# daultanigaurav/AI-BASED-FRAME-INTERPOLATION

Hardware: AMD Instinct MI355X
Metric: interpolated frames/sec at 1080p (higher is better)
Workload: dtype bf16

## Files before the change

ai_based_frame_interpolation_amd/_native.py:

```python
from __future__ import annotations

import ctypes
import os
import subprocess

import torch

_PKG = os.path.dirname(os.path.abspath(__file__))
LIB_PATH = os.environ.get("FIUNET_LIB") or os.path.join(_PKG, "libfiunet_hip.so")
CSRC = os.path.join(_PKG, "csrc")

ABI_VERSION = 8
ABI_MIN_COMPAT = 4
FP32, BF16, BF16X2, FP16 = 0, 1, 2, 3
OPT_UNFUSED, OPT_KEEP_ALL, OPT_GATHER_UPSAMPLE = 1, 2, 16
OPT_RNE_WEIGHTS, OPT_NO_DITHER = 32, 64
WEIGHT_PREPS = ("host", "device")
YUV_MPEG2, YUV_BT709, YUV_FULL_RANGE, YUV_BT2020 = 1, 2, 4, 8

SYMBOLS = (
    "fiunet_abi_version", "fiunet_last_error_string", "fiunet_create", "fiunet_destroy",
    "fiunet_set_options", "fiunet_load_weights", "fiunet_load_weights_device", "fiunet_prepare_precision", "fiunet_workspace_bytes", "fiunet_forward",
    "fiunet_min_unsplit_batch",
    "fiunet_forward_strip",
    "fiunet_workspace_bytes_u8", "fiunet_forward_u8", "fiunet_forward_u8_strided", "fiunet_preprocess_u8",
    "fiunet_postprocess_u8", "fiunet_debug_read_activation", "fiunet_profile_enable",
    "fiunet_profile_read", "fiunet_metrics_workspace_bytes", "fiunet_psnr_u8", "fiunet_ssim_u8",
    "fiunet_ssim_gauss_workspace_bytes", "fiunet_ssim_gauss_f32",
    "fiunet_plane_metrics_workspace_bytes", "fiunet_plane_psnr", "fiunet_plane_ssim",
    "fiunet_interleaved_psnr", "fiunet_stepped_ssim",
    "fiunet_yuv420_to_rgb_u8", "fiunet_rgb_to_yuv420_u8", "fiunet_workspace_bytes_yuv420", "fiunet_forward_yuv420",
# ... 794 lines not shown
```

ai_based_frame_interpolation_amd/csrc/conv3x3_mfma.hip.h:

```cpp
#pragma once
#include "conv_common.hip.h"

namespace fiunet {

template <typename T, int BN, int TH, int TW, int MODE, int EPI>
__global__ __launch_bounds__(256, conv_occupancy(BN, TH, TW, ConvTile<BN, TH, TW, MODE>::LDS_BYTES)) void conv3x3_mfma_kernel(const ConvArgs a)
{
    using Tile = ConvTile<BN, TH, TW, MODE>;
    constexpr int PL = Elem<T>::PL;
    constexpr int TWP = Tile::TWP, THP = Tile::THP;
    constexpr int WAVES_C = BN / 64, WAVES_P = 4 / WAVES_C;
    constexpr int FR = TW / 16;
    constexpr int NF = conv_wave_frags(BN, TH, TW);
    constexpr int ROWS_W = NF / FR;
    static_assert(NF == 8 || NF == 4, "wave tile must be 64 couts x 128 or 64 pixels");
    static_assert(TH == ROWS_W * WAVES_P && ROWS_W * FR == NF, "tile does not split over the waves");
    static_assert(EPI != EPI_POOL || ROWS_W % 2 == 0, "pooled epilogue: a wave owns whole row pairs");
    static_assert(Tile::LDS_BYTES * conv_occupancy(BN, TH, TW, Tile::LDS_BYTES) <= 160 * 1024, "LDS per CU");
    constexpr int HNC = EPI == EPI_HEAD ? 1 : (EPI == EPI_HEAD3 ? 3 : 0);
    static_assert(HNC == 0 || BN == 64, "fused head needs all 64 couts in one wave");
    static_assert(MODE == SRC_DIRECT || MODE == SRC_CONCAT_UP || MODE == SRC_STEM || MODE == SRC_DIRECT_X2 ||
                  MODE == SRC_STEM_X2, "pooling is fused into the producer");
    constexpr bool X2 = src_is_x2(MODE);
    constexpr bool STEM = src_is_stem(MODE);
    constexpr bool DIRECT = MODE == SRC_DIRECT || MODE == SRC_DIRECT_X2;
    static_assert(!X2 || std::is_same_v<T, __bf16>, "two-piece operands are bf16");
    static_assert(!STEM || (sizeof(T) == 2 && BN == 64), "fused stem: 2-byte output (bf16 / fp16), 64 couts");

    extern __shared__ __attribute__((aligned(16))) char smem[];
    char* const lds_in = smem;
    char* const lds_w = smem + Tile::IN_BYTES;
// ... 30 lines not shown
#define STAMP(slot) do {} while (0)
#define STAMP_UP(slot) do {} while (0)
#define PSTAMP(slot) do {} while (0)
#endif
    f32x4 acc[4][NF];
    conv_acc_init<T, BN, TH, TW, EPI>(a, acc, ct, wc, lc);
#ifdef FIUNET_STAMP_PROLOG
    asm volatile("" :: "v"(acc[3][NF - 1][3]), "v"(acc[0][0][0]));
#endif
    PSTAMP(9);

    const int a_off = (wc * 64 + l15) * 64 + ((lc ^ swz(l15)) << 4);
    int b_off[3];
#pragma unroll
    for (int kx = 0; kx < 3; ++kx)
        b_off[kx] = (wp * ROWS_W * TWP + kx + l15) * 64 + ((lc ^ swz(kx + l15)) << 4);

    const int nplanes_real = (a.C0 + a.C1) / PL;
    const int nplanes_all = X2 ? 3 * nplanes_real : nplanes_real;
    const int p0 = a.C0 / PL;
    const int pbeg = split * nplanes_all / ksplit, pend = (split + 1) * nplanes_all / ksplit;
    const int nsteps = (pend - pbeg) * 3;
    const char* wbase = (const char*)a.wgt + (size_t)ct * BN * 64;

    constexpr int NW = Tile::W_BYTES / 1024 / 4;
    static_assert(BN % 16 == 0, "a weight piece must not straddle two taps");
    const unsigned w_lane_off = (unsigned)((lane >> 2) * 64 + (((lane & 3) ^ swz(lane >> 2)) << 4));
    auto issue_w = [&](int step) __attribute__((always_inline)) {
        const int lp = step / 3, kx = step - lp * 3;
        int pl = pbeg + lp;
        if constexpr (X2) {
// ... 12 lines not shown
#ifndef FIUNET_DIAG_FREE_PROLOGUE
    issue_w(0);
#endif
#ifdef FIUNET_DIAG_NO_WSTREAM
    if (nsteps > 1) issue_w(1);
#endif
    PSTAMP(10);

    constexpr int NPIECE = THP * TWP / 16;
    static_assert(THP * TWP % 16 == 0, "in-tile must be a whole number of 1-KiB pieces");
    const int aH = a.H, aW = a.W;
    const char* const dma_src = (const char*)a.src0 + (size_t)b * a.H * a.W * a.C0 * sizeof(T) * (X2 ? 2 : 1);
    const char* const dma_src1 = DIRECT && a.C1 > 0
                                     ? (const char*)a.src1 + (size_t)b * a.H * a.W * a.C1 * sizeof(T) * (X2 ? 2 : 1) : nullptr;
    constexpr bool HOIST = (MODE == SRC_DIRECT && BN == 128 && EPI == EPI_PLAIN) ||
                           (NF == 4 && DIRECT);
    constexpr bool ROLL = sizeof(T) == 2 && FR == 2 && (!epi_is_splitk(EPI) || NF == 4);
    constexpr int NPW = (NPIECE + 3) / 4;
    unsigned in_off[HOIST ? NPW : 1];
    const unsigned plane_bytes = (unsigned)(aH * aW) * 64u;
    unsigned pm_lin0 = 0, pm_valid = 0, pm_wrap = 0;
    static_assert(NPW <= 32, "one mask bit per piece of a wave");
    constexpr int PM_DY = 64 / TWP, PM_DX = 64 % TWP;
    const unsigned pm_dlin = (unsigned)(PM_DY * aW + PM_DX) * 64u, pm_dwrap = (unsigned)(aW - TWP) * 64u;
    if constexpr (!STEM) {
        const int row0 = wave * 16 + (lane >> 2);
        int py = row0 / TWP, px = row0 - py * TWP;
        int y = y0 - 1 + py, x = x0 - 1 + px;
        pm_lin0 = (unsigned)(y * aW + x) * 64u + (((lane & 3) ^ swz(row0)) << 4);
        unsigned lin = pm_lin0;
#pragma unroll
        for (int jj = 0; jj < NPW; ++jj) {
// ... 380 lines not shown
#endif
            const char* wcur = lds_w + (step & 1) * Tile::W_STRIDE + a_off;
            constexpr bool EARLY_OK = ROLL && DIRECT;
            bool early = false;
            if constexpr (EARLY_OK)
                early = kx == 2 && gather_next && (DIRECT || plane + 1 < p0);
            if constexpr (ROLL) {
                uint4 xb[ROWS_W + 2][FR];
                auto load_row = [&](int i) __attribute__((always_inline)) {
#pragma unroll
                    for (int f = 0; f < FR; ++f)
                        xb[i][f] = *reinterpret_cast<const uint4*>(lds_in + b_off[kx] + (i * TWP + f * 16) * 64);
                };
#pragma unroll
                for (int i = 0; i < ROWS_W; ++i) load_row(i);
#pragma unroll
                for (int ky = 0; ky < 3; ++ky) {
                    uint4 wa[4];
#pragma unroll
                    for (int m = 0; m < 4; ++m)
                        wa[m] = *reinterpret_cast<const uint4*>(wcur + (ky * BN + m * 16) * 64);
                    if (ky < 2) load_row(ROWS_W + ky);
                    if (ky == 1 && early) {
                        __syncthreads();
                        gather_plane(plane + 1, step & 1, false);
                    }
#pragma unroll
                    for (int m = 0; m < 4; ++m)
#pragma unroll
                        for (int n = 0; n < NF; ++n) mma_chunk<T>(acc[m][n], wa[m], xb[n / FR + ky][n % FR]);
                }
            } else {
#pragma unroll
                for (int ky = 0; ky < 3; ++ky) {
                    asm volatile("" ::: "memory");
                    uint4 wa[4], xb[NF];
#pragma unroll
                    for (int m = 0; m < 4; ++m)
                        wa[m] = *reinterpret_cast<const uint4*>(wcur + (ky * BN + m * 16) * 64);
#pragma unroll
                    for (int n = 0; n < NF; ++n)
                        xb[n] = *reinterpret_cast<const uint4*>(
                            lds_in + b_off[kx] + (((n / FR) + ky) * TWP + (n % FR) * 16) * 64);
#pragma unroll
                    for (int m = 0; m < 4; ++m)
// ... 23 lines not shown

#ifdef FIUNET_CLOCK
    {
        asm volatile("" :: "v"(acc[3][NF - 1][3]));
        __builtin_amdgcn_sched_barrier(0);
        const unsigned long long ck_t1 = __builtin_amdgcn_s_memtime(), ck_r1 = __builtin_amdgcn_s_memrealtime();
        const unsigned st_idx = blockIdx.x * 4u + (unsigned)wave;
        if (a.stamp && lane == 0 && st_idx < a.stamp_cap) {
            unsigned long long* rec = a.stamp + (size_t)st_idx * 16;
            rec[0] = ck_t1 - ck_t0;
            rec[1] = ck_r1 - ck_r0;
            rec[8] = 1ull;
        }
    }
#endif
    conv_epilogue<T, BN, TH, TW, EPI, X2>(a, acc, b, y0, x0, ct, split, wc, wp, l15, lc);
#ifdef FIUNET_STAMP
    STAMP(5);
    st_sum[0] = st_prev - st_t0;
    const unsigned st_idx = blockIdx.x * 4u + (unsigned)wave;
    if (a.stamp && lane == 0 && st_idx < a.stamp_cap) {
        unsigned long long* rec = a.stamp + (size_t)st_idx * 16;
#pragma unroll
        for (int k = 0; k < 16; ++k) rec[k] = k == 8 ? 1ull : st_sum[k];
    }
#endif
}

template <typename T, int BN, int TH, int TW, int EPI, bool X2>
__global__ __launch_bounds__(64) void splitk_finalize_tile_kernel(const ConvArgs a)
{
// ... 56 lines not shown
```

ai_based_frame_interpolation_amd/csrc/conv_common.hip.h:

```cpp
#pragma once
#include <hip/hip_runtime.h>
#include <stdint.h>
#include <type_traits>

namespace fiunet {

typedef __attribute__((ext_vector_type(4))) float f32x4;
typedef __attribute__((ext_vector_type(8))) __bf16 bf16x8;
typedef __attribute__((ext_vector_type(8))) _Float16 f16x8;

enum SrcMode { SRC_DIRECT = 0, SRC_POOL = 1 , SRC_CONCAT_UP = 2,
               SRC_STEM = 3 ,
               SRC_DIRECT_X2 = 4,
               SRC_STEM_X2 = 5 };
constexpr bool src_is_stem(int mode) { return mode == SRC_STEM || mode == SRC_STEM_X2; }
constexpr bool src_is_x2(int mode) { return mode == SRC_DIRECT_X2 || mode == SRC_STEM_X2; }

__device__ __forceinline__ size_t blk_off(int plane, int y, int x, int H, int W)
{
    return (((size_t)plane * H + y) * W + x) * 64;
}

struct ConvArgs {
    const void* src0;
// ... 374 lines not shown
    static constexpr int TAB_OFF = PATCH_OFF + ((PATCH_BYTES + 15) / 16) * 16;
    static constexpr int TAB_BYTES = MODE == SRC_CONCAT_UP ? ((THP + TW + 2) * 16 + 255) / 256 * 256 : 0;
    static constexpr int STEMW_OFF = TAB_OFF + TAB_BYTES;
    static constexpr int STEMW_BYTES = src_is_stem(MODE) ? 4096 : 0;
    static constexpr int LDS_BYTES = STEMW_OFF + STEMW_BYTES;
    static_assert(LDS_BYTES <= 80 * 1024, "two workgroups must fit in the CU's 160 KiB of LDS");
    static_assert(!src_is_stem(MODE) || LDS_BYTES <= 63 * 1280, "fused-stem kernel: stay below 64 LDS granules");
};

constexpr int conv_wave_frags(int BN, int TH, int TW) { return TH * TW / 16 / (4 / (BN / 64)); }
constexpr int conv_occupancy(int BN, int TH, int TW, int lds_bytes = 0)
{
    return conv_wave_frags(BN, TH, TW) == 4 && lds_bytes * 3 <= 160 * 1024 ? 3 : 2;
}


__device__ __forceinline__ int conv_block_remap()
{
    const int nblk = gridDim.x, bid = blockIdx.x;
    const int q = nblk >> 3, r = nblk & 7, xcd = bid & 7;
    return (xcd < r ? xcd * (q + 1) : r * (q + 1) + (xcd - r) * q) + (bid >> 3);
}

struct ConvTileId { int ct, b, ty, tx; };
__device__ __forceinline__ ConvTileId conv_tile_decode(const ConvArgs& a, int t)
{
    ConvTileId d;
    d.ct = t % a.nct; t /= a.nct;
    d.tx = t % a.tilesX; t /= a.tilesX;
    d.ty = t % a.tilesY;
// ... 18 lines not shown
            const float4 sh = *reinterpret_cast<const float4*>(a.shift + ct * BN + wc * 64 + conv_cout_ofs<T>(m, lc));
            v = f32x4{sh.x, sh.y, sh.z, sh.w};
        }
#pragma unroll
        for (int n = 0; n < NF; ++n) acc[m][n] = v;
    }
}

__device__ __forceinline__ unsigned relu_pk_bf16(unsigned p) { return pk_max_i16(p, 0u); }
__device__ __forceinline__ void relu_fma(float& sum, float x, float lo, float w)
{
    float t;
    asm("v_max_f32 %1, %3, %2\n\tv_fmac_f32 %0, %1, %4" : "+v"(sum), "=&v"(t) : "v"(x), "v"(lo), "v"(w));
}

template <typename T, int BN, int TH, int TW, int EPI, bool X2 = false>
__device__ __forceinline__ void conv_epilogue(const ConvArgs& a, f32x4 (&acc)[4][conv_wave_frags(BN, TH, TW)],
                                              int b, int y0, int x0, int ct, int split, int wc, int wp,
                                              int l15, int lc)
{
    constexpr int PL = Elem<T>::PL;
    constexpr int FR = TW / 16;
    constexpr int NF = conv_wave_frags(BN, TH, TW);
    constexpr int ROWS_W = NF / FR;
    constexpr int HNC = EPI == EPI_HEAD ? 1 : (EPI == EPI_HEAD3 ? 3 : 0);
    const int aH = a.H, aW = a.W;
    constexpr bool PERM = sizeof(T) == 2;
    const int wbase_c = ct * BN + wc * 64;
    if constexpr (epi_is_splitk(EPI)) {
        const int tile = (((b * a.tilesY) + y0 / TH) * a.tilesX + x0 / TW) * a.nct + ct;
        const int ntile = a.B * a.tilesY * a.tilesX * a.nct;
        const int wave = wp * (BN / 64) + wc;
        float4* o = reinterpret_cast<float4*>(a.kslab) + ((((size_t)split * ntile + tile) * 4 + wave) * (4 * NF)) * 64 + (lc * 16 + l15);
#pragma unroll
        for (int m = 0; m < 4; ++m)
#pragma unroll
            for (int n = 0; n < NF; ++n)
                o[(m * NF + n) * 64] = make_float4(acc[m][n][0], acc[m][n][1], acc[m][n][2], acc[m][n][3]);
        return;
    }
    float hw[HNC > 0 ? HNC : 1][4][4];
// ... 29 lines not shown
#pragma unroll
                for (int m = 0; m < 4; ++m)
#pragma unroll
                    for (int j = 0; j < 4; ++j) relu_fma(sum, acc[m][n][j], floor_v, hw[c][m][j]);
                hs[n] = sum;
            }
            if constexpr (NF == 4) {
                float full[NF];
#pragma unroll
                for (int n = 0; n < NF; ++n) {
                    const float p = hs[n] + __shfl_xor(hs[n], 16);
                    full[n] = p + __shfl_xor(p, 32);
                }
                const float mine = lc == 0 ? full[0] : (lc == 1 ? full[1] : (lc == 2 ? full[2] : full[3]));
                const int n = lc;
                const int y = y0 + wp * ROWS_W + n / FR;
                const int x = x0 + (n % FR) * 16 + l15;
                if (y < aH && x < aW) {
                    const size_t o = (size_t)b * a.head_img_stride + ((size_t)c * aH + y) * aW + x;
                    if (a.head_out_u8) a.head_out_u8[o] = postprocess_u8_value(mine + hb[c]);
                    else a.head_out[o] = mine + hb[c];
                }
            } else {
                float t[4], u[2];
#pragma unroll
                for (int i = 0; i < 4; ++i) {
                    const auto r = __builtin_amdgcn_permlane16_swap(__float_as_uint(hs[i]), __float_as_uint(hs[(i + 4) % NF]), false, false);
                    t[i] = __uint_as_float(r[0]) + __uint_as_float(r[1]);
                }
#pragma unroll
                for (int j = 0; j < 2; ++j) {
                    const auto r = __builtin_amdgcn_permlane32_swap(__float_as_uint(t[j]), __float_as_uint(t[j + 2]), false, false);
                    u[j] = __uint_as_float(r[0]) + __uint_as_float(r[1]);
                }
#pragma unroll
                for (int j = 0; j < 2; ++j) {
                    const int n = nb + j;
                    const int y = y0 + wp * ROWS_W + n / FR;
                    const int x = x0 + (n % FR) * 16 + l15;
                    if (y < aH && x < aW) {
                        const size_t o = (size_t)b * a.head_img_stride + ((size_t)c * aH + y) * aW + x;
                        if (a.head_out_u8) a.head_out_u8[o] = postprocess_u8_value(u[j] + hb[c]);
                        else a.head_out[o] = u[j] + hb[c];
                    }
                }
            }
        }
    }
    if constexpr (X2) {
        static_assert(std::is_same_v<T, __bf16>, "the two-piece epilogue belongs to the bf16 kernels");
        if (HNC > 0 && !a.dst) return;
        const size_t ps = (size_t)aH * aW * 64;
        const int npo = a.Cout / 32;
        const size_t blk = (size_t)npo * ps;
// ... 2 lines not shown
        const size_t pps = (size_t)pH2 * pW2 * 64, pblk = (size_t)npo * pps;
        char* const pimg = EPI == EPI_POOL ? (char*)a.pool_dst + (size_t)b * 2 * pblk + (size_t)(wbase_c / 32) * pps + lc * 16
                                           : nullptr;
        auto put = [&](char* o, size_t block_bytes, const float (&v)[8]) __attribute__((always_inline)) {
            unsigned h[4], l[4];
#pragma unroll
            for (int i = 0; i < 4; ++i) {
                h[i] = pack_bf16x2_pk(v[2 * i], v[2 * i + 1]);
                l[i] = pack_bf16x2_pk(v[2 * i] - __uint_as_float(h[i] << 16), v[2 * i + 1] - __uint_as_float(h[i] & 0xffff0000u));
            }
            *reinterpret_cast<uint4*>(o) = make_uint4(h[0], h[1], h[2], h[3]);
            *reinterpret_cast<uint4*>(o + block_bytes) = make_uint4(l[0], l[1], l[2], l[3]);
        };
#pragma unroll
        for (int n = 0; n < NF; ++n) {
            const int y = y0 + wp * ROWS_W + n / FR;
            const int x = x0 + (n % FR) * 16 + l15;
            if (y < aH && x < aW) {
#pragma unroll
                for (int g = 0; g < 2; ++g) {
                    float v[8];
#pragma unroll
                    for (int j = 0; j < 4; ++j) {
                        v[j] = a.relu ? fmaxf(acc[2 * g][n][j], 0.f) : acc[2 * g][n][j];
                        v[4 + j] = a.relu ? fmaxf(acc[2 * g + 1][n][j], 0.f) : acc[2 * g + 1][n][j];
                    }
                    put(img + (size_t)(y * aW + x) * 64 + g * ps, blk, v);
                }
            }
        }
        if constexpr (EPI == EPI_POOL) {
#pragma unroll
            for (int n = 0; n < NF; ++n) {
                if (((n / FR) & 1) != 0) continue;
                const int y = y0 + wp * ROWS_W + n / FR;
                const int x = x0 + (n % FR) * 16 + l15;
                const int py = y >> 1, px = x >> 1;
                const bool okp = (py < pH2) && (px < pW2) && ((l15 & 1) == 0);
#pragma unroll
                for (int g = 0; g < 2; ++g) {
                    float v[8];
#pragma unroll
                    for (int h = 0; h < 2; ++h)
#pragma unroll
                        for (int j = 0; j < 4; ++j) {
                            const float cm = fmaxf(acc[2 * g + h][n][j], acc[2 * g + h][n + FR][j]);
                            float r = fmaxf(cm, __uint_as_float(dpp_swap_pairs(__float_as_uint(cm))));
                            if (a.relu) r = fmaxf(r, 0.f);
                            v[4 * h + j] = r;
                        }
                    if (okp) put(pimg + (size_t)(min(py, pH2 - 1) * pW2 + min(px, pW2 - 1)) * 64 + g * pps, pblk, v);
                }
            }
        }
        return;
    }
    if constexpr (EPI == EPI_POOL && PERM) {
#pragma unroll
        for (int n = 0; n < NF; ++n) {
            if (((n / FR) & 1) != 0) continue;
            uint4 pk[2][2];
#pragma unroll
            for (int r = 0; r < 2; ++r) {
                const int nn = n + r * FR;
                const int y = y0 + wp * ROWS_W + nn / FR;
                const int x = x0 + (nn % FR) * 16 + l15;
                const bool ok = (y < aH) && (x < aW);
                char* o = out_img + (size_t)(y * aW + x) * 64;
#pragma unroll
                for (int g = 0; g < 2; ++g) {
                    uint4 v = make_uint4(pack2_pk<T>(acc[2 * g][nn][0], acc[2 * g][nn][1]),
                                         pack2_pk<T>(acc[2 * g][nn][2], acc[2 * g][nn][3]),
                                         pack2_pk<T>(acc[2 * g + 1][nn][0], acc[2 * g + 1][nn][1]),
                                         pack2_pk<T>(acc[2 * g + 1][nn][2], acc[2 * g + 1][nn][3]));
                    if (a.relu) v = make_uint4(relu_pk_bf16(v.x), relu_pk_bf16(v.y), relu_pk_bf16(v.z), relu_pk_bf16(v.w));
                    pk[r][g] = v;
                    if (ok && out_img) *reinterpret_cast<uint4*>(o + g * plane_stride) = v;
                }
            }
            const int y = y0 + wp * ROWS_W + n / FR;
            const int x = x0 + (n % FR) * 16 + l15;
            const int py = y >> 1, px = x >> 1;
            const bool okp = (py < pH) && (px < pW) && ((l15 & 1) == 0);
            char* o = pool_img + (size_t)(min(py, pH - 1) * pW + min(px, pW - 1)) * 64;
#pragma unroll
            for (int g = 0; g < 2; ++g) {
                const uint4 t = pk[0][g], u = pk[1][g];
                const unsigned c0 = pk_max_i16(t.x, u.x), c1 = pk_max_i16(t.y, u.y);
                const unsigned c2 = pk_max_i16(t.z, u.z), c3 = pk_max_i16(t.w, u.w);
                const uint4 m = make_uint4(pk_max_i16(c0, dpp_swap_pairs(c0)), pk_max_i16(c1, dpp_swap_pairs(c1)),
                                           pk_max_i16(c2, dpp_swap_pairs(c2)), pk_max_i16(c3, dpp_swap_pairs(c3)));
                if (okp) *reinterpret_cast<uint4*>(o + g * pplane_stride) = m;
            }
        }
        return;
    }
#pragma unroll
    for (int n = 0; n < NF; ++n) {
        const int y = y0 + wp * ROWS_W + n / FR;
        const int x = x0 + (n % FR) * 16 + l15;
        const bool ok = (y < aH) && (x < aW);
        if (ok && out_img) {
            char* o = out_img + (size_t)(y * aW + x) * 64;
            if constexpr (PERM) {
#pragma unroll
                for (int g = 0; g < 2; ++g) {
                    uint4 pk = make_uint4(pack2<T>(acc[2 * g][n][0], acc[2 * g][n][1]),
                                          pack2<T>(acc[2 * g][n][2], acc[2 * g][n][3]),
                                          pack2<T>(acc[2 * g + 1][n][0], acc[2 * g + 1][n][1]),
                                          pack2<T>(acc[2 * g + 1][n][2], acc[2 * g + 1][n][3]));
                    if (a.relu) pk = make_uint4(relu_pk_bf16(pk.x), relu_pk_bf16(pk.y), relu_pk_bf16(pk.z), relu_pk_bf16(pk.w));
                    *reinterpret_cast<uint4*>(o + g * plane_stride) = pk;
                }
            } else {
#pragma unroll
                for (int m = 0; m < 4; ++m) {
                    float4 v = make_float4(acc[m][n][0], acc[m][n][1], acc[m][n][2], acc[m][n][3]);
                    if (a.relu) v = make_float4(fmaxf(v.x, 0.f), fmaxf(v.y, 0.f), fmaxf(v.z, 0.f), fmaxf(v.w, 0.f));
                    *reinterpret_cast<float4*>(o + m * plane_stride) = v;
                }
            }
        }
    }
    if (EPI == EPI_POOL) {
#pragma unroll
        for (int n = 0; n < NF; ++n) {
            if (((n / FR) & 1) != 0) continue;
            const int y = y0 + wp * ROWS_W + n / FR;
            const int x = x0 + (n % FR) * 16 + l15;
            const int py = y >> 1, px = x >> 1;
            const bool okp = (py < pH) && (px < pW) && ((l15 & 1) == 0);
            char* o = pool_img + (size_t)(min(py, pH - 1) * pW + min(px, pW - 1)) * 64;
            if constexpr (!PERM) {
#pragma unroll
                for (int m = 0; m < 4; ++m) {
                    float r[4];
#pragma unroll
                    for (int j = 0; j < 4; ++j) {
                        const float cm = fmaxf(acc[m][n][j], acc[m][n + FR][j]);
                        r[j] = fmaxf(cm, __uint_as_float(dpp_swap_pairs(__float_as_uint(cm))));
                        if (a.relu) r[j] = fmaxf(r[j], 0.f);
                    }
                    if (okp) *reinterpret_cast<float4*>(o + m * pplane_stride) = make_float4(r[0], r[1], r[2], r[3]);
                }
// ... 24 lines not shown
```

ai_based_frame_interpolation_amd/csrc/conv_launch.hip.h:

```cpp
#pragma once
#include "fiunet_internal.h"
#include "conv3x3_kwave.hip.h"

#include <atomic>
#include <cstdio>

namespace fiunet {
namespace {

template <auto Kernel>
int launch_lds(const char* name, long long nblk, int lds, const ConvArgs& a, hipStream_t s)
{
    if (name_out()) *name_out() = name;
    if (nblk <= 0 || nblk > 0x7fffffffLL) return fail(FIUNET_ERR_INVALID_ARG, "conv grid too large");
    static std::atomic<bool> lds_attr_set[64];
    int dev = 0;
    HIP_TRY(hipGetDevice(&dev));
    if (dev >= 0 && dev < 64 && !lds_attr_set[dev].load(std::memory_order_acquire)) {
        HIP_TRY(hipFuncSetAttribute(reinterpret_cast<const void*>(Kernel), hipFuncAttributeMaxDynamicSharedMemorySize, lds));
        lds_attr_set[dev].store(true, std::memory_order_release);
    }
    hipLaunchKernelGGL(Kernel, dim3((unsigned)nblk), dim3(256), lds, s, a);
    HIP_TRY(hipGetLastError());
    return FIUNET_OK;
}

template <typename T, int BN, int TH, int TW, int MODE, int EPI>
int launch_conv_cfg(ConvArgs a, hipStream_t s)
{
    char name[128] = "";
    if (name_out())
        std::snprintf(name, sizeof name, "conv3x3_mfma_kernel<%s,%d,%d,%d,%d,%d>", elem_name<T>(), BN, TH, TW,
                      MODE, EPI);
    a.tilesX = (a.W + TW - 1) / TW;
    a.tilesY = (a.H + TH - 1) / TH;
    a.nct = a.Cout / BN;
    const long long nblk = (long long)a.B * a.tilesX * a.tilesY * a.nct * (epi_is_splitk(EPI) ? a.ksplit : 1);
    return launch_lds<&conv3x3_mfma_kernel<T, BN, TH, TW, MODE, EPI>>(name, nblk, ConvTile<BN, TH, TW, MODE>::LDS_BYTES, a, s);
}

template <typename T, int EPI, bool X2> int launch_kwave(ConvArgs a, hipStream_t s)
{
    using Tile = KWaveTile;
    char name[96] = "";
    if (name_out())
        std::snprintf(name, sizeof name, "conv3x3_kwave_kernel<%s%s,64,2,32,%d>+kwave4", elem_name<T>(), X2 ? "x2" : "", EPI);
    a.tilesX = (a.W + Tile::TW - 1) / Tile::TW;
    a.tilesY = (a.H + Tile::TH - 1) / Tile::TH;
    a.nct = a.Cout / Tile::BN;
    return launch_lds<&conv3x3_kwave_kernel<EPI, X2, T>>(name, (long long)a.B * a.tilesX * a.tilesY * a.nct, Tile::LDS_BYTES, a, s);
}

template <typename T, int BN, int TH, int TW, int MODE, int EPI>
// ... 14 lines not shown
            if (name_out()) *name_out() += "+splitk" + std::to_string(ksplit);
            return FIUNET_OK;
        }
    }
    return launch_conv_cfg<T, BN, TH, TW, MODE, EPI>(a, s);
}

template <typename T, int MODE, int EPI> int launch_conv_shape(const ConvArgs& a, const ConvCfg& cfg, hipStream_t s)
{
    if (a.Cout != 64 && a.Cout % 128 != 0) return fail(FIUNET_ERR_INVALID_ARG, "Cout must be 64 or k*128");
    if ((EPI == EPI_HEAD || EPI == EPI_HEAD3) && a.Cout != 64) return fail(FIUNET_ERR_INVALID_ARG, "fused head needs Cout == 64");
    if constexpr ((MODE == SRC_DIRECT || MODE == SRC_DIRECT_X2) && (EPI == EPI_PLAIN || EPI == EPI_POOL)) {
        if (cfg.kwave) return launch_kwave<T, EPI, MODE == SRC_DIRECT_X2>(a, s);
    }
    if (cfg.small) return launch_conv_maybe_split<T, 64, 8, 32, MODE, EPI>(a, s, cfg.ksplit);
    if (a.Cout == 64) {
        const bool wide = prefer_wide(a.H, a.W, 16, 32, 32, 16);
        return wide ? launch_conv_maybe_split<T, 64, 16, 32, MODE, EPI>(a, s, cfg.ksplit)
                    : launch_conv_maybe_split<T, 64, 32, 16, MODE, EPI>(a, s, cfg.ksplit);
    }
    if constexpr (EPI != EPI_HEAD && EPI != EPI_HEAD3) {
        const bool wide = prefer_wide(a.H, a.W, 8, 32, 16, 16);
        return wide ? launch_conv_maybe_split<T, 128, 8, 32, MODE, EPI>(a, s, cfg.ksplit)
                    : launch_conv_maybe_split<T, 128, 16, 16, MODE, EPI>(a, s, cfg.ksplit);
    }
    return fail(FIUNET_ERR_INVALID_ARG, "fused head needs Cout == 64");
}

}

template <typename T> int launch_conv(const ConvArgs& a, int mode, int epi, const ConvCfg& cfg, hipStream_t s)
{
    constexpr int PL = Elem<T>::PL;
    if (a.C0 % PL || a.C1 % PL) return fail(FIUNET_ERR_INVALID_ARG, "channels not a plane multiple");
    if (mode == SRC_CONCAT_UP && epi == EPI_PLAIN) return launch_conv_shape<T, SRC_CONCAT_UP, EPI_PLAIN>(a, cfg, s);
    if (mode == SRC_DIRECT && epi == EPI_PLAIN) return launch_conv_shape<T, SRC_DIRECT, EPI_PLAIN>(a, cfg, s);
    if (mode == SRC_DIRECT && epi == EPI_HEAD) return launch_conv_shape<T, SRC_DIRECT, EPI_HEAD>(a, cfg, s);
// ... 15 lines not shown
```

ai_based_frame_interpolation_amd/csrc/fiunet.hip:

```cpp
#include "fiunet_internal.h"
#include "pointwise.hip.h"
#include "weights.hip.h"

#include <cmath>
#include <cstdio>
#include <cstring>
#include <map>

using namespace fiunet;

namespace {

thread_local std::string g_err;

thread_local std::string* g_name_out = nullptr;

}

namespace fiunet {

std::string& last_error() { return g_err; }

int fail(int code, const std::string& msg)
{
// ... 234 lines not shown
            if (!n.bilinear) st.form = FORM_CONCAT_CONVT;
            else if (x2) st.form = FORM_CONCAT_UP;
            else if (unfused) st.form = FORM_CONCAT_UPCAT;
            else st.form = !gather_up && materialise_up(precision, B, h, w, cin, cout) ? FORM_CONCAT_UP : FORM_CONCAT_GATHER;
        }
        if (kPoolOut[i] >= 0 && !unfused) st.epi = EPI_POOL;
        if (i == NCONV - 1 && !unfused) st.epi = n.cf == 1 ? EPI_HEAD : EPI_HEAD3;
        st.slab = i != NCONV - 1;
        st.stored = !(i == NCONV - 1 && st.epi != EPI_PLAIN && !keep_all);
        const bool stem = st.form == FORM_STEM, gather = st.form == FORM_CONCAT_GATHER, direct = !stem && !gather;
        const bool plain_or_pool = st.epi == EPI_PLAIN || st.epi == EPI_POOL;
        const bool as_gather = st.form == FORM_CONCAT_UPCAT && fp32 && !fp32_concat_takes_kwave(B, h, w, cin, cout);
        st.cfg = choose_conv_cfg(fp32, x2, B, h, w, cin, cout, !stem && plain_or_pool && st.slab,
                                 (n.force_tile ? n.force_tile[i] : 0) - 1, stem || !n.force_ksplit ? 0 : n.force_ksplit[i],
                                 direct && plain_or_pool && !as_gather, direct || (gather && cout >= 256), gather || as_gather);
    }
}

struct Plan {
    StageLaunch st[NCONV];
    int hs[5], ws[5];
    size_t act_off[NCONV];
    size_t pool_off[4];
    size_t scratch_off;
    size_t up_off[NCONV];
    size_t slab_off;
    size_t total;
};

enum BufKind { BUF_ACT = 0, BUF_POOL = 1, BUF_UP = 2, BUF_SCRATCH = 3, BUF_SLAB = 4 };
// ... 904 lines not shown
    NetDesc n;
    n.cf = frame_channels;
    n.bilinear = bilinear != 0;
    n.cout = n.bilinear ? kCoutBil : kCoutCT;
    n.flags = flags;
    n.stem_w = frame_channels == 1;
    StageLaunch L[NCONV];
    plan_stages(n, precision, B, H, W, L);
    const StageLaunch& st = L[stage];
    out[0] = st.cfg.small; out[1] = st.cfg.ksplit; out[2] = st.cfg.kwave;
    out[3] = stage > 0 && (st.form == FORM_CONCAT_UP || st.form == FORM_CONCAT_CONVT);
    out[4] = st.form; out[5] = st.epi;
    return FIUNET_OK;
}

int fiunet_debug_plan(int frame_channels, int bilinear, unsigned flags, int precision, int B, int H, int W,
                      long long* records , int capacity, int* n_records, unsigned long long* total)
{
    if (!records || capacity < 0 || !n_records || !total || (frame_channels != 1 && frame_channels != 3) || B < 1 || H < 16 ||
        W < 16 || !valid_precision(precision))
        return fail(FIUNET_ERR_INVALID_ARG, "fiunet_debug_plan: bad arguments");
    NetDesc n;
    n.cf = frame_channels;
    n.bilinear = bilinear != 0;
    n.cout = n.bilinear ? kCoutBil : kCoutCT;
    n.flags = flags;
    n.stem_w = frame_channels == 1;
    Plan p;
    std::vector<PlanBuf> bufs;
    if (!make_plan(n, B, H, W, precision, p, &bufs))
// ... 128 lines not shown
```

ai_based_frame_interpolation_amd/csrc/fiunet_internal.h:

```cpp
#pragma once
#include "../../include/fiunet.h"

#include <hip/hip_runtime.h>

#include <algorithm>
#include <string>
#include <type_traits>
#include <vector>

#pragma GCC visibility push(hidden)

namespace fiunet {

struct ConvArgs;

std::string& last_error();
int fail(int code, const std::string& msg);

#define HIP_TRY(expr)                                                                     \
    do {                                                                                  \
        hipError_t e_ = (expr);                                                           \
        if (e_ != hipSuccess)                                                             \
            return fail(FIUNET_ERR_HIP, std::string(#expr) + ": " + hipGetErrorString(e_)); \
    } while (0)
// ... 24 lines not shown
inline unsigned grid_for(size_t n) { return (unsigned)std::min<size_t>((n + 255) / 256, 256 * 32); }

int zero_fill_async(void* p, size_t bytes, hipStream_t s);

inline long long padded_area(int H, int W, int TH, int TW)
{
    return (long long)((H + TH - 1) / TH) * TH * ((W + TW - 1) / TW) * TW;
}

inline bool prefer_wide(int H, int W, int THw, int TWw, int THn, int TWn)
{
    const long long wide = padded_area(H, W, THw, TWw), narrow = padded_area(H, W, THn, TWn);
    return wide * 32 <= narrow * 33;
}

struct ConvCfg { bool small; int ksplit; bool kwave = false; };

std::string* name_out();

template <typename T> int launch_conv(const ConvArgs& a, int mode, int epi, const ConvCfg& cfg, hipStream_t s);
extern template int launch_conv<float>(const ConvArgs&, int, int, const ConvCfg&, hipStream_t);
extern template int launch_conv<_Float16>(const ConvArgs&, int, int, const ConvCfg&, hipStream_t);
extern template int launch_conv<__bf16>(const ConvArgs&, int, int, const ConvCfg&, hipStream_t);
int launch_conv_x2(const ConvArgs& a, int mode, int epi, const ConvCfg& cfg, hipStream_t s);

}

#pragma GCC visibility pop

struct fiunet_ctx {
    int device = 0;
// ... 25 lines not shown
```

ai_based_frame_interpolation_amd/unet.py:

```python
from __future__ import annotations

import contextlib
import os

import torch
import torch.nn as nn

from . import _native

_ENCODER = (("down1", 64, 128), ("down2", 128, 256), ("down3", 256, 512), ("down4", 512, 512))
_DECODER = (("up1", 1024, 256), ("up2", 512, 128), ("up3", 256, 64), ("up4", 128, 64))
_ENCODER_CT = (("down1", 64, 128), ("down2", 128, 256), ("down3", 256, 512), ("down4", 512, 1024))
_DECODER_CT = (("up1", 1024, 512), ("up2", 512, 256), ("up3", 256, 128), ("up4", 128, 64))

TAP_CHANNELS = (64, 64, 128, 128, 256, 256, 512, 512, 512, 512, 512, 256, 256, 128, 128, 64, 64, 64)
TAP_CHANNELS_CT = (64, 64, 128, 128, 256, 256, 512, 512, 1024, 1024, 512, 512, 256, 256, 128, 128, 64, 64)
TAP_LEVEL = (0, 0, 1, 1, 2, 2, 3, 3, 4, 4, 3, 3, 2, 2, 1, 1, 0, 0)
TAP_NAMES = tuple(
    f"{p}.double_conv.{c}"
    for p in ("unet.inc", "unet.down1.maxpool_conv.1", "unet.down2.maxpool_conv.1",
              "unet.down3.maxpool_conv.1", "unet.down4.maxpool_conv.1", "unet.up1.conv",
              "unet.up2.conv", "unet.up3.conv", "unet.up4.conv")
    for c in (0, 3))

# ... 128 lines not shown
        new = self.__class__.__new__(self.__class__)
        memo[id(self)] = new
        for k, v in self.__getstate__().items():
            new.__dict__[k] = copy.deepcopy(v, memo)
        return new

    def load_state_dict(self, *a, **k):
        self._ctx_dirty = True
        self._tracked = None
        return super().load_state_dict(*a, **k)

    def refresh_weights(self):
        self._ctx_dirty = True

    def set_options(self, *, unfused: bool = False, keep_all: bool = False, gather_upsample: bool = False,
                    rne_weights: bool = False, no_dither: bool = False):
        old = self._options
        self._options = ((_native.OPT_UNFUSED if unfused else 0) | (_native.OPT_KEEP_ALL if keep_all else 0)
                         | (_native.OPT_GATHER_UPSAMPLE if gather_upsample else 0)
                         | (_native.OPT_RNE_WEIGHTS if rne_weights else 0)
                         | (_native.OPT_NO_DITHER if no_dither else 0))
        if (old ^ self._options) & _native.OPT_RNE_WEIGHTS:
            self._ctx_dirty = True
        if self._ctx is not None:
            self._ctx.set_options(self._options)

    def _ctx_or_none_set_options(self):
        if self._ctx is not None:
            self._ctx.set_options(self._options)

    def _context(self, device: torch.device) -> "_native.Context":
        idx = device.index if device.index is not None else torch.cuda.current_device()
        if self._ctx is None or self._ctx.device_index != idx:
            if self._ctx is not None:
                self._ctx.close()
            self._ctx = _native.Context(idx, self.frame_channels, self.unet.bilinear)
# ... 322 lines not shown
```

include/fiunet.h:

```cpp
#ifndef FIUNET_H
#define FIUNET_H

#include <stddef.h>
#include <stdint.h>

#ifdef __cplusplus
extern "C" {
#endif

#define FIUNET_ABI_VERSION 8

enum fiunet_status {
    FIUNET_OK = 0,
    FIUNET_ERR_INVALID_ARG = 1,
    FIUNET_ERR_BAD_SHAPE = 2,
    FIUNET_ERR_MISSING_WEIGHT = 3,
    FIUNET_ERR_NOT_LOADED = 4,
    FIUNET_ERR_WORKSPACE = 5,
    FIUNET_ERR_HIP = 6,
    FIUNET_ERR_UNSUPPORTED = 7
};

enum fiunet_precision {
    FIUNET_FP32 = 0,
    FIUNET_BF16 = 1,
    FIUNET_BF16X2 = 2,
    FIUNET_FP16 = 3
};

enum fiunet_option {
    FIUNET_OPT_UNFUSED = 1,
    FIUNET_OPT_KEEP_ALL = 2,
    FIUNET_OPT_RNE_WEIGHTS = 32,
    FIUNET_OPT_NO_DITHER = 64,
    FIUNET_OPT_GATHER_UPSAMPLE = 16
};

typedef struct fiunet_ctx fiunet_ctx;

int fiunet_create(fiunet_ctx** out_ctx, int device_id, int frame_channels, int bilinear);

int fiunet_destroy(fiunet_ctx* ctx);

int fiunet_set_options(fiunet_ctx* ctx, unsigned flags);

int fiunet_load_weights(fiunet_ctx* ctx, int n, const char* const* names,
                        const float* const* host_ptrs, const int64_t* numels);

int fiunet_load_weights_device(fiunet_ctx* ctx, int n, const char* const* names,
                               const float* const* device_ptrs, const int64_t* numels, void* stream);
// ... 265 lines not shown
```

Before: 537.0.

## Add strip wave shape for direct bf16 conv kernels with pinned weight prefetch

Introduces a WAVE_STRIP geometry in which each wave owns an 8-row by 16-pixel column strip of a 32-wide tile instead of full-width rows. It is enabled by default for selected direct bf16/fp16 stages (pool/head epilogues at Cout 64, plain/pool at 128). In the strip path, the next ky's weight fragments are double-buffered into registers, with a sched_barrier after each ky step. The aim is to change input-fragment reuse and overlap LDS weight reads with MFMAs. The cost is more register pressure, a new template variant, and a WIDE_WAVES option to opt out.

```diff
diff --git a/ai_based_frame_interpolation_amd/_native.py b/ai_based_frame_interpolation_amd/_native.py
--- a/ai_based_frame_interpolation_amd/_native.py
+++ b/ai_based_frame_interpolation_amd/_native.py
@@ -15,6 +15,7 @@
 FP32, BF16, BF16X2, FP16 = 0, 1, 2, 3
 OPT_UNFUSED, OPT_KEEP_ALL, OPT_GATHER_UPSAMPLE = 1, 2, 16
 OPT_RNE_WEIGHTS, OPT_NO_DITHER = 32, 64
+OPT_WIDE_WAVES = 128
 WEIGHT_PREPS = ("host", "device")
 YUV_MPEG2, YUV_BT709, YUV_FULL_RANGE, YUV_BT2020 = 1, 2, 4, 8
 
diff --git a/ai_based_frame_interpolation_amd/csrc/conv3x3_mfma.hip.h b/ai_based_frame_interpolation_amd/csrc/conv3x3_mfma.hip.h
--- a/ai_based_frame_interpolation_amd/csrc/conv3x3_mfma.hip.h
+++ b/ai_based_frame_interpolation_amd/csrc/conv3x3_mfma.hip.h
@@ -3,18 +3,20 @@
 
 namespace fiunet {
 
-template <typename T, int BN, int TH, int TW, int MODE, int EPI>
+template <typename T, int BN, int TH, int TW, int MODE, int EPI, int SHAPE = WAVE_WIDE>
 __global__ __launch_bounds__(256, conv_occupancy(BN, TH, TW, ConvTile<BN, TH, TW, MODE>::LDS_BYTES)) void conv3x3_mfma_kernel(const ConvArgs a)
 {
     using Tile = ConvTile<BN, TH, TW, MODE>;
+    using Geom = WaveGeom<BN, TH, TW, SHAPE>;
     constexpr int PL = Elem<T>::PL;
     constexpr int TWP = Tile::TWP, THP = Tile::THP;
     constexpr int WAVES_C = BN / 64, WAVES_P = 4 / WAVES_C;
-    constexpr int FR = TW / 16;
+    constexpr int FR = Geom::FR;
     constexpr int NF = conv_wave_frags(BN, TH, TW);
-    constexpr int ROWS_W = NF / FR;
+    constexpr int ROWS_W = Geom::ROWS_W;
     static_assert(NF == 8 || NF == 4, "wave tile must be 64 couts x 128 or 64 pixels");
-    static_assert(TH == ROWS_W * WAVES_P && ROWS_W * FR == NF, "tile does not split over the waves");
+    static_assert(TH * Geom::COLS == ROWS_W * WAVES_P && ROWS_W * FR == NF, "tile does not split over the waves");
+    static_assert(SHAPE == WAVE_WIDE || (MODE == SRC_DIRECT && sizeof(T) == 2 && !epi_is_splitk(EPI)), "strip wave shape: direct bf16 / fp16 kernels");
     static_assert(EPI != EPI_POOL || ROWS_W % 2 == 0, "pooled epilogue: a wave owns whole row pairs");
     static_assert(Tile::LDS_BYTES * conv_occupancy(BN, TH, TW, Tile::LDS_BYTES) <= 160 * 1024, "LDS per CU");
     constexpr int HNC = EPI == EPI_HEAD ? 1 : (EPI == EPI_HEAD3 ? 3 : 0);
@@ -75,7 +77,7 @@
     int b_off[3];
 #pragma unroll
     for (int kx = 0; kx < 3; ++kx)
-        b_off[kx] = (wp * ROWS_W * TWP + kx + l15) * 64 + ((lc ^ swz(kx + l15)) << 4);
+        b_off[kx] = (Geom::row0(wp) * TWP + Geom::col0(wp) + kx + l15) * 64 + ((lc ^ swz(kx + l15)) << 4);
 
     const int nplanes_real = (a.C0 + a.C1) / PL;
     const int nplanes_all = X2 ? 3 * nplanes_real : nplanes_real;
@@ -118,8 +120,9 @@
     const char* const dma_src1 = DIRECT && a.C1 > 0
                                      ? (const char*)a.src1 + (size_t)b * a.H * a.W * a.C1 * sizeof(T) * (X2 ? 2 : 1) : nullptr;
     constexpr bool HOIST = (MODE == SRC_DIRECT && BN == 128 && EPI == EPI_PLAIN) ||
+                           (SHAPE == WAVE_STRIP && ((BN == 128 && EPI == EPI_POOL) || (BN == 64 && EPI == EPI_HEAD))) ||
                            (NF == 4 && DIRECT);
-    constexpr bool ROLL = sizeof(T) == 2 && FR == 2 && (!epi_is_splitk(EPI) || NF == 4);
+    constexpr bool ROLL = sizeof(T) == 2 && TW == 32 && (!epi_is_splitk(EPI) || NF == 4);
     constexpr int NPW = (NPIECE + 3) / 4;
     unsigned in_off[HOIST ? NPW : 1];
     const unsigned plane_bytes = (unsigned)(aH * aW) * 64u;
@@ -530,12 +533,28 @@
                 };
 #pragma unroll
                 for (int i = 0; i < ROWS_W; ++i) load_row(i);
+                constexpr bool PINNED = SHAPE == WAVE_STRIP;
+                uint4 wnext[PINNED ? 2 : 1][4];
+                if constexpr (PINNED) {
+#pragma unroll
+                    for (int m = 0; m < 4; ++m) wnext[0][m] = *reinterpret_cast<const uint4*>(wcur + (m * 16) * 64);
+                }
 #pragma unroll
                 for (int ky = 0; ky < 3; ++ky) {
                     uint4 wa[4];
-#pragma unroll
-                    for (int m = 0; m < 4; ++m)
-                        wa[m] = *reinterpret_cast<const uint4*>(wcur + (ky * BN + m * 16) * 64);
+                    if constexpr (PINNED) {
+                        if (ky < 2) {
+#pragma unroll
+                            for (int m = 0; m < 4; ++m)
+                                wnext[(ky + 1) & 1][m] = *reinterpret_cast<const uint4*>(wcur + ((ky + 1) * BN + m * 16) * 64);
+                        }
+#pragma unroll
+                        for (int m = 0; m < 4; ++m) wa[m] = wnext[ky & 1][m];
+                    } else {
+#pragma unroll
+                        for (int m = 0; m < 4; ++m)
+                            wa[m] = *reinterpret_cast<const uint4*>(wcur + (ky * BN + m * 16) * 64);
+                    }
                     if (ky < 2) load_row(ROWS_W + ky);
                     if (ky == 1 && early) {
                         __syncthreads();
@@ -545,6 +564,7 @@
                     for (int m = 0; m < 4; ++m)
 #pragma unroll
                         for (int n = 0; n < NF; ++n) mma_chunk<T>(acc[m][n], wa[m], xb[n / FR + ky][n % FR]);
+                    if constexpr (PINNED) __builtin_amdgcn_sched_barrier(0);
                 }
             } else {
 #pragma unroll
@@ -598,7 +618,7 @@
         }
     }
 #endif
-    conv_epilogue<T, BN, TH, TW, EPI, X2>(a, acc, b, y0, x0, ct, split, wc, wp, l15, lc);
+    conv_epilogue<T, BN, TH, TW, EPI, X2, SHAPE>(a, acc, b, y0, x0, ct, split, wc, wp, l15, lc);
 #ifdef FIUNET_STAMP
     STAMP(5);
     st_sum[0] = st_prev - st_t0;
diff --git a/ai_based_frame_interpolation_amd/csrc/conv_common.hip.h b/ai_based_frame_interpolation_amd/csrc/conv_common.hip.h
--- a/ai_based_frame_interpolation_amd/csrc/conv_common.hip.h
+++ b/ai_based_frame_interpolation_amd/csrc/conv_common.hip.h
@@ -412,6 +412,19 @@
     return conv_wave_frags(BN, TH, TW) == 4 && lds_bytes * 3 <= 160 * 1024 ? 3 : 2;
 }
 
+enum WaveShape { WAVE_WIDE = 0, WAVE_STRIP = 1 };
+template <int BN, int TH, int TW, int SHAPE> struct WaveGeom {
+    static constexpr int NF = conv_wave_frags(BN, TH, TW);
+    static constexpr int FR = SHAPE == WAVE_STRIP ? 1 : TW / 16;
+    static constexpr int ROWS_W = NF / FR;
+    static constexpr int COLS = TW / 16 / FR;
+    static_assert(SHAPE == WAVE_WIDE || SHAPE == WAVE_STRIP, "unknown wave shape");
+    static_assert(SHAPE != WAVE_STRIP || (TW == 32 && NF == 8), "strips: 8 rows x 16 pixels of a 32-wide tile");
+    static_assert(ROWS_W * FR == NF && TH * COLS == ROWS_W * (4 / (BN / 64)), "tile does not split over the waves");
+    __device__ static __forceinline__ int row0(int wp) { return (wp / COLS) * ROWS_W; }
+    __device__ static __forceinline__ int col0(int wp) { return (wp % COLS) * FR * 16; }
+};
+
 
 __device__ __forceinline__ int conv_block_remap()
 {
@@ -460,17 +473,19 @@
     asm("v_max_f32 %1, %3, %2\n\tv_fmac_f32 %0, %1, %4" : "+v"(sum), "=&v"(t) : "v"(x), "v"(lo), "v"(w));
 }
 
-template <typename T, int BN, int TH, int TW, int EPI, bool X2 = false>
+template <typename T, int BN, int TH, int TW, int EPI, bool X2 = false, int SHAPE = WAVE_WIDE>
 __device__ __forceinline__ void conv_epilogue(const ConvArgs& a, f32x4 (&acc)[4][conv_wave_frags(BN, TH, TW)],
                                               int b, int y0, int x0, int ct, int split, int wc, int wp,
                                               int l15, int lc)
 {
+    using Geom = WaveGeom<BN, TH, TW, SHAPE>;
     constexpr int PL = Elem<T>::PL;
-    constexpr int FR = TW / 16;
-    constexpr int NF = conv_wave_frags(BN, TH, TW);
-    constexpr int ROWS_W = NF / FR;
+    constexpr int FR = Geom::FR;
+    constexpr int NF = Geom::NF;
+    static_assert(!epi_is_splitk(EPI) || SHAPE == WAVE_WIDE, "the split-K slab and its reduction keep the wide shape");
     constexpr int HNC = EPI == EPI_HEAD ? 1 : (EPI == EPI_HEAD3 ? 3 : 0);
     const int aH = a.H, aW = a.W;
+    const int yw = y0 + Geom::row0(wp), xw = x0 + Geom::col0(wp);
     constexpr bool PERM = sizeof(T) == 2;
     const int wbase_c = ct * BN + wc * 64;
     if constexpr (epi_is_splitk(EPI)) {
@@ -530,8 +545,8 @@
                 }
                 const float mine = lc == 0 ? full[0] : (lc == 1 ? full[1] : (lc == 2 ? full[2] : full[3]));
                 const int n = lc;
-                const int y = y0 + wp * ROWS_W + n / FR;
-                const int x = x0 + (n % FR) * 16 + l15;
+                const int y = yw + n / FR;
+                const int x = xw + (n % FR) * 16 + l15;
                 if (y < aH && x < aW) {
                     const size_t o = (size_t)b * a.head_img_stride + ((size_t)c * aH + y) * aW + x;
                     if (a.head_out_u8) a.head_out_u8[o] = postprocess_u8_value(mine + hb[c]);
@@ -552,8 +567,8 @@
 #pragma unroll
                 for (int j = 0; j < 2; ++j) {
                     const int n = nb + j;
-                    const int y = y0 + wp * ROWS_W + n / FR;
-                    const int x = x0 + (n % FR) * 16 + l15;
+                    const int y = yw + n / FR;
+                    const int x = xw + (n % FR) * 16 + l15;
                     if (y < aH && x < aW) {
                         const size_t o = (size_t)b * a.head_img_stride + ((size_t)c * aH + y) * aW + x;
                         if (a.head_out_u8) a.head_out_u8[o] = postprocess_u8_value(u[j] + hb[c]);
@@ -586,8 +601,8 @@
         };
 #pragma unroll
         for (int n = 0; n < NF; ++n) {
-            const int y = y0 + wp * ROWS_W + n / FR;
-            const int x = x0 + (n % FR) * 16 + l15;
+            const int y = yw + n / FR;
+            const int x = xw + (n % FR) * 16 + l15;
             if (y < aH && x < aW) {
 #pragma unroll
                 for (int g = 0; g < 2; ++g) {
@@ -605,8 +620,8 @@
 #pragma unroll
             for (int n = 0; n < NF; ++n) {
                 if (((n / FR) & 1) != 0) continue;
-                const int y = y0 + wp * ROWS_W + n / FR;
-                const int x = x0 + (n % FR) * 16 + l15;
+                const int y = yw + n / FR;
+                const int x = xw + (n % FR) * 16 + l15;
                 const int py = y >> 1, px = x >> 1;
                 const bool okp = (py < pH2) && (px < pW2) && ((l15 & 1) == 0);
 #pragma unroll
@@ -635,8 +650,8 @@
 #pragma unroll
             for (int r = 0; r < 2; ++r) {
                 const int nn = n + r * FR;
-                const int y = y0 + wp * ROWS_W + nn / FR;
-                const int x = x0 + (nn % FR) * 16 + l15;
+                const int y = yw + nn / FR;
+                const int x = xw + (nn % FR) * 16 + l15;
                 const bool ok = (y < aH) && (x < aW);
                 char* o = out_img + (size_t)(y * aW + x) * 64;
 #pragma unroll
@@ -650,8 +665,8 @@
                     if (ok && out_img) *reinterpret_cast<uint4*>(o + g * plane_stride) = v;
                 }
             }
-            const int y = y0 + wp * ROWS_W + n / FR;
-            const int x = x0 + (n % FR) * 16 + l15;
+            const int y = yw + n / FR;
+            const int x = xw + (n % FR) * 16 + l15;
             const int py = y >> 1, px = x >> 1;
             const bool okp = (py < pH) && (px < pW) && ((l15 & 1) == 0);
             char* o = pool_img + (size_t)(min(py, pH - 1) * pW + min(px, pW - 1)) * 64;
@@ -669,8 +684,8 @@
     }
 #pragma unroll
     for (int n = 0; n < NF; ++n) {
-        const int y = y0 + wp * ROWS_W + n / FR;
-        const int x = x0 + (n % FR) * 16 + l15;
+        const int y = yw + n / FR;
+        const int x = xw + (n % FR) * 16 + l15;
         const bool ok = (y < aH) && (x < aW);
         if (ok && out_img) {
             char* o = out_img + (size_t)(y * aW + x) * 64;
@@ -698,8 +713,8 @@
 #pragma unroll
         for (int n = 0; n < NF; ++n) {
             if (((n / FR) & 1) != 0) continue;
-            const int y = y0 + wp * ROWS_W + n / FR;
-            const int x = x0 + (n % FR) * 16 + l15;
+            const int y = yw + n / FR;
+            const int x = xw + (n % FR) * 16 + l15;
             const int py = y >> 1, px = x >> 1;
             const bool okp = (py < pH) && (px < pW) && ((l15 & 1) == 0);
             char* o = pool_img + (size_t)(min(py, pH - 1) * pW + min(px, pW - 1)) * 64;
diff --git a/ai_based_frame_interpolation_amd/csrc/conv_launch.hip.h b/ai_based_frame_interpolation_amd/csrc/conv_launch.hip.h
--- a/ai_based_frame_interpolation_amd/csrc/conv_launch.hip.h
+++ b/ai_based_frame_interpolation_amd/csrc/conv_launch.hip.h
@@ -25,18 +25,18 @@
     return FIUNET_OK;
 }
 
-template <typename T, int BN, int TH, int TW, int MODE, int EPI>
+template <typename T, int BN, int TH, int TW, int MODE, int EPI, int SHAPE = WAVE_WIDE>
 int launch_conv_cfg(ConvArgs a, hipStream_t s)
 {
     char name[128] = "";
     if (name_out())
-        std::snprintf(name, sizeof name, "conv3x3_mfma_kernel<%s,%d,%d,%d,%d,%d>", elem_name<T>(), BN, TH, TW,
-                      MODE, EPI);
+        std::snprintf(name, sizeof name, "conv3x3_mfma_kernel<%s,%d,%d,%d,%d,%d%s>", elem_name<T>(), BN, TH, TW,
+                      MODE, EPI, SHAPE == WAVE_STRIP ? ",strip" : "");
     a.tilesX = (a.W + TW - 1) / TW;
     a.tilesY = (a.H + TH - 1) / TH;
     a.nct = a.Cout / BN;
     const long long nblk = (long long)a.B * a.tilesX * a.tilesY * a.nct * (epi_is_splitk(EPI) ? a.ksplit : 1);
-    return launch_lds<&conv3x3_mfma_kernel<T, BN, TH, TW, MODE, EPI>>(name, nblk, ConvTile<BN, TH, TW, MODE>::LDS_BYTES, a, s);
+    return launch_lds<&conv3x3_mfma_kernel<T, BN, TH, TW, MODE, EPI, SHAPE>>(name, nblk, ConvTile<BN, TH, TW, MODE>::LDS_BYTES, a, s);
 }
 
 template <typename T, int EPI, bool X2> int launch_kwave(ConvArgs a, hipStream_t s)
@@ -81,13 +81,25 @@
         if (cfg.kwave) return launch_kwave<T, EPI, MODE == SRC_DIRECT_X2>(a, s);
     }
     if (cfg.small) return launch_conv_maybe_split<T, 64, 8, 32, MODE, EPI>(a, s, cfg.ksplit);
+    const bool wide = tuned_tile_is_wide(a.H, a.W, a.Cout);
+    if (cfg.strip) {
+        if constexpr (sizeof(T) == 2 && MODE == SRC_DIRECT) {
+            if (wide && cfg.ksplit <= 1) {
+                if constexpr (conv_strip_pays(64, EPI)) {
+                    if (a.Cout == 64) return launch_conv_cfg<T, 64, 16, 32, MODE, EPI, WAVE_STRIP>(a, s);
+                }
+                if constexpr (conv_strip_pays(128, EPI)) {
+                    if (a.Cout != 64) return launch_conv_cfg<T, 128, 8, 32, MODE, EPI, WAVE_STRIP>(a, s);
+                }
+            }
+        }
+        return fail(FIUNET_ERR_INVALID_ARG, "internal: strip wave shape asked of a launch that has none");
+    }
     if (a.Cout == 64) {
-        const bool wide = prefer_wide(a.H, a.W, 16, 32, 32, 16);
         return wide ? launch_conv_maybe_split<T, 64, 16, 32, MODE, EPI>(a, s, cfg.ksplit)
                     : launch_conv_maybe_split<T, 64, 32, 16, MODE, EPI>(a, s, cfg.ksplit);
     }
     if constexpr (EPI != EPI_HEAD && EPI != EPI_HEAD3) {
-        const bool wide = prefer_wide(a.H, a.W, 8, 32, 16, 16);
         return wide ? launch_conv_maybe_split<T, 128, 8, 32, MODE, EPI>(a, s, cfg.ksplit)
                     : launch_conv_maybe_split<T, 128, 16, 16, MODE, EPI>(a, s, cfg.ksplit);
     }
diff --git a/ai_based_frame_interpolation_amd/csrc/fiunet.hip b/ai_based_frame_interpolation_amd/csrc/fiunet.hip
--- a/ai_based_frame_interpolation_amd/csrc/fiunet.hip
+++ b/ai_based_frame_interpolation_amd/csrc/fiunet.hip
@@ -272,6 +272,8 @@
         st.cfg = choose_conv_cfg(fp32, x2, B, h, w, cin, cout, !stem && plain_or_pool && st.slab,
                                  (n.force_tile ? n.force_tile[i] : 0) - 1, stem || !n.force_ksplit ? 0 : n.force_ksplit[i],
                                  direct && plain_or_pool && !as_gather, direct || (gather && cout >= 256), gather || as_gather);
+        st.cfg.strip = conv_wave_strip(precision == FIUNET_BF16 || precision == FIUNET_FP16, direct, st.cfg, h, w, cout, st.epi,
+                                       (n.flags & FIUNET_OPT_WIDE_WAVES) != 0);
     }
 }
 
@@ -1206,6 +1208,24 @@
     return FIUNET_OK;
 }
 
+int fiunet_debug_stage_wave_shape(int frame_channels, int bilinear, unsigned flags, int precision, int B, int H, int W,
+                                  int stage, int* out)
+{
+    if (!out || (frame_channels != 1 && frame_channels != 3) || B < 1 || H < 16 || W < 16 || stage < 1 || stage >= NCONV ||
+        !valid_precision(precision))
+        return fail(FIUNET_ERR_INVALID_ARG, "fiunet_debug_stage_wave_shape: bad arguments");
+    NetDesc n;
+    n.cf = frame_channels;
+    n.bilinear = bilinear != 0;
+    n.cout = n.bilinear ? kCoutBil : kCoutCT;
+    n.flags = flags;
+    n.stem_w = frame_channels == 1;
+    StageLaunch L[NCONV];
+    plan_stages(n, precision, B, H, W, L);
+    *out = L[stage].cfg.strip;
+    return FIUNET_OK;
+}
+
 int fiunet_debug_plan(int frame_channels, int bilinear, unsigned flags, int precision, int B, int H, int W,
                       long long* records , int capacity, int* n_records, unsigned long long* total)
 {
diff --git a/ai_based_frame_interpolation_amd/csrc/fiunet_internal.h b/ai_based_frame_interpolation_amd/csrc/fiunet_internal.h
--- a/ai_based_frame_interpolation_amd/csrc/fiunet_internal.h
+++ b/ai_based_frame_interpolation_amd/csrc/fiunet_internal.h
@@ -62,7 +62,22 @@
     return wide * 32 <= narrow * 33;
 }
 
-struct ConvCfg { bool small; int ksplit; bool kwave = false; };
+inline bool tuned_tile_is_wide(int H, int W, int Cout)
+{
+    return Cout == 64 ? prefer_wide(H, W, 16, 32, 32, 16) : prefer_wide(H, W, 8, 32, 16, 16);
+}
+
+struct ConvCfg { bool small; int ksplit; bool kwave = false; bool strip = false; };
+
+constexpr bool conv_strip_pays(int Cout, int epi)
+{
+    return Cout == 64 ? (epi == 1 || epi == 2 || epi == 3) : (epi == 0 || epi == 2);
+}
+inline bool conv_wave_strip(bool two_byte, bool direct, const ConvCfg& cfg, int H, int W, int Cout, int epi, bool force_wide)
+{
+    return !force_wide && two_byte && direct && !cfg.small && !cfg.kwave && cfg.ksplit <= 1 &&
+           tuned_tile_is_wide(H, W, Cout) && conv_strip_pays(Cout, epi);
+}
 
 std::string* name_out();
 
diff --git a/ai_based_frame_interpolation_amd/unet.py b/ai_based_frame_interpolation_amd/unet.py
--- a/ai_based_frame_interpolation_amd/unet.py
+++ b/ai_based_frame_interpolation_amd/unet.py
@@ -166,12 +166,13 @@
         self._ctx_dirty = True
 
     def set_options(self, *, unfused: bool = False, keep_all: bool = False, gather_upsample: bool = False,
-                    rne_weights: bool = False, no_dither: bool = False):
+                    rne_weights: bool = False, no_dither: bool = False, wide_waves: bool = False):
         old = self._options
         self._options = ((_native.OPT_UNFUSED if unfused else 0) | (_native.OPT_KEEP_ALL if keep_all else 0)
                          | (_native.OPT_GATHER_UPSAMPLE if gather_upsample else 0)
                          | (_native.OPT_RNE_WEIGHTS if rne_weights else 0)
-                         | (_native.OPT_NO_DITHER if no_dither else 0))
+                         | (_native.OPT_NO_DITHER if no_dither else 0)
+                         | (_native.OPT_WIDE_WAVES if wide_waves else 0))
         if (old ^ self._options) & _native.OPT_RNE_WEIGHTS:
             self._ctx_dirty = True
         if self._ctx is not None:
diff --git a/include/fiunet.h b/include/fiunet.h
--- a/include/fiunet.h
+++ b/include/fiunet.h
@@ -33,7 +33,8 @@
     FIUNET_OPT_KEEP_ALL = 2,
     FIUNET_OPT_RNE_WEIGHTS = 32,
     FIUNET_OPT_NO_DITHER = 64,
-    FIUNET_OPT_GATHER_UPSAMPLE = 16
+    FIUNET_OPT_GATHER_UPSAMPLE = 16,
+    FIUNET_OPT_WIDE_WAVES = 128
 };
 
 typedef struct fiunet_ctx fiunet_ctx;
```

Result: no change. 541.4, median of 4 (+0.8%).
